# rosielab/emojivoice

Measured on AMD Instinct MI355X. Metric: audio_seconds_per_second, higher is better.
Workload: dtype f32 (deep layers: operand = two block-scaled fp16 pieces, product = 3 fp16 products on the fp16 MFMA, f32 accumulate); 1 GPU; config2: batch 64 x 516-frame (5.99 s) utterances per GPU, 10 Euler steps + HiFi-GAN V1, 22.05 kHz; global_batch=64, frames=516, ode_steps=10, parallelism=dp1, collective=none, batch_pipeline=cfm(i+1) || hifigan(i) on two streams, 2 pipeline(s) in flight

## Files before the change

emojivoice_amd/_lib.py:

```python
from __future__ import annotations

import ctypes as C
import os
import subprocess
from typing import Dict, Optional

import numpy as np
import torch

_HERE = os.path.dirname(os.path.abspath(__file__))
LIB_PATH = os.environ.get("EV_LIB_PATH") or os.path.join(_HERE, "lib", "libemojivoice_hip.so")
CSRC = os.path.join(_HERE, "csrc")

EXPORTS = [
    "ev_abi_version", "ev_create", "ev_destroy", "ev_last_error", "ev_load_estimator", "ev_load_vocoder", "ev_load_vocoder_cfg", "ev_load_text_encoder", "ev_text_encoder",
    "ev_text_encoder_status", "ev_stft_magnitude", "ev_denoise", "ev_align", "ev_dbg_conv_bench",
    "ev_workspace_bytes", "ev_cfm_decode", "ev_estimator", "ev_hifigan", "ev_profile_enable", "ev_profile_read", "ev_profile_read_split", "ev_dbg_last_cfg", "ev_set_arithmetic", "ev_get_arithmetic",
    "ev_op_conv1d", "ev_op_groupnorm_mish", "ev_op_groupnorm_mish2", "ev_op_conv_groupnorm", "ev_op_layernorm", "ev_op_split_pieces", "ev_op_attention", "ev_op_ln_mlp", "ev_set_mrf_streams_max",
    "ev_cfm_decode2", "ev_reserve", "ev_alloc_count", "ev_dbg_sk_stats", "ev_op_attn_out", "ev_dbg_set_amax", "ev_dbg_set_attn_h16", "ev_dbg_set_chain", "ev_dbg_sk_taken",
    "ev_load_mel_basis", "ev_mel_spectrogram",
    "ev_maximum_path", "ev_log_prior", "ev_mas_align",
    "ev_estimator_rows", "ev_cfm_loss",
    "ev_load_resampler", "ev_resample", "ev_mel_stats",
    "ev_trim_bounds", "ev_trim_apply",
    "ev_pitch_yin", "ev_dtw",
    "ev_loudness",
    "ev_pyin_observe", "ev_pyin_decode",
    "ev_op_attention2", "ev_op_attn_out2",
    "ev_load_stoi", "ev_stoi",
    "ev_load_stft_dist", "ev_stft_dist",
]


class EvLibraryError(RuntimeError):
# ... 116 lines not shown
    lib.ev_stft_dist.argtypes = [vp, vp, vp, vp, i32, i32, C.c_double, vp, vp, vp, vp]
    lib.ev_maximum_path.argtypes = [vp, vp, vp, vp, i32, i32, i32, vp, vp, vp]
    lib.ev_log_prior.argtypes = [vp, vp, vp, i32, i32, i32, vp, vp]
    lib.ev_mas_align.argtypes = [vp, vp, vp, vp, vp, i32, i32, i32, vp, vp, vp, vp, vp]
    lib.ev_profile_enable.argtypes = [vp, i32]
    lib.ev_profile_read.argtypes = [vp, C.POINTER(C.c_double), C.POINTER(C.c_double), C.POINTER(C.c_int64), i32]
    lib.ev_profile_read_split.argtypes = [vp, C.POINTER(C.c_double), C.POINTER(C.c_double), C.POINTER(C.c_int64)]
    lib.ev_dbg_last_cfg.argtypes = [vp]
    lib.ev_set_arithmetic.argtypes = [vp, i32]
    lib.ev_get_arithmetic.argtypes = [vp]
    lib.ev_dbg_set_amax.argtypes = [vp, i32]
    lib.ev_dbg_set_attn_h16.argtypes = [vp, i32]
    lib.ev_dbg_set_chain.argtypes = [vp, i32]
    lib.ev_dbg_sk_taken.argtypes = [vp]
    lib.ev_dbg_sk_taken.restype = C.c_int64
    lib.ev_op_conv1d.argtypes = [vp, vp, vp, vp, i32, i32, i32, i32, i32, i32, i32, i32, i32, f32, vp, vp]
    lib.ev_op_groupnorm_mish.argtypes = [vp, vp, vp, vp, vp, i32, i32, i32, i32, vp, vp]
    lib.ev_op_groupnorm_mish2.argtypes = [vp, vp, vp, vp, vp, i32, i32, i32, i32, i32, vp, i32, vp, vp, vp]
    lib.ev_op_conv_groupnorm.argtypes = [vp, vp, vp, vp, i32, i32, i32, vp, vp, vp, i32, vp, vp, vp, vp, vp, C.POINTER(C.c_int), vp]
    lib.ev_op_layernorm.argtypes = [vp, vp, vp, vp, i32, i32, vp, vp]
    lib.ev_op_split_pieces.argtypes = [vp, vp, i32, vp, vp]
    lib.ev_op_attention.argtypes = [vp, vp, vp, i32, i32, i32, vp, vp]
    lib.ev_op_attn_out.argtypes = [vp, vp, vp, i32, i32, vp, vp, vp, vp]
    lib.ev_op_attention2.argtypes = [vp, vp, vp, i32, i32, i32, i32, i32, i32, vp, C.POINTER(C.c_int), vp]
    lib.ev_op_attn_out2.argtypes = [vp, vp, vp, i32, i32, i32, i32, vp, vp, f32, f32, f32, vp, C.POINTER(C.c_int), vp]
    lib.ev_op_ln_mlp.argtypes = [vp, vp, vp, vp, vp, vp, vp, vp, vp, vp, vp, i32, i32, i32, vp, vp]
    for n in EXPORTS:
        getattr(lib, n)
    _lib = lib
    return lib
# ... 548 lines not shown
        self._check(self.lib.ev_op_split_pieces(self.h, x.data_ptr(), x.numel(), out.data_ptr(), _stream_ptr()), "ev_op_split_pieces")
        return out

    def set_arithmetic(self, bf16_products: int):
        self._check(self.lib.ev_set_arithmetic(self.h, int(bf16_products)), "ev_set_arithmetic")

    def set_amax(self, on: bool) -> None:
        self._check(self.lib.ev_dbg_set_amax(self.h, int(bool(on))), "ev_dbg_set_amax")

    def set_attn_h16(self, on: bool) -> None:
        self._check(self.lib.ev_dbg_set_attn_h16(self.h, int(bool(on))), "ev_dbg_set_attn_h16")

    def set_chain(self, on: bool) -> None:
        self._check(self.lib.ev_dbg_set_chain(self.h, int(bool(on))), "ev_dbg_set_chain")

    def arithmetic(self) -> int:
        return int(self.lib.ev_get_arithmetic(self.h))

    def last_cfg(self) -> int:
        return int(self.lib.ev_dbg_last_cfg(self.h))

    def profile_read_split(self):
        ms, fl, n = C.c_double(), C.c_double(), C.c_int64()
        self._check(self.lib.ev_profile_read_split(self.h, C.byref(ms), C.byref(fl), C.byref(n)), "ev_profile_read_split")
        return ms.value, fl.value, n.value

    def profile_read(self, reset: bool = True):
        ms, fl, n = C.c_double(), C.c_double(), C.c_int64()
        self._check(self.lib.ev_profile_read(self.h, C.byref(ms), C.byref(fl), C.byref(n), int(reset)), "ev_profile_read")
        return ms.value, fl.value, n.value
# ... 148 lines not shown
```

emojivoice_amd/csrc/ev_engine.hip:

```cpp
#include "ev_kernels.h"
#include "../../include/emojivoice.h"

#include <math.h>
#include <stdlib.h>
#include <stdarg.h>
#include <stdio.h>
#include <string.h>

#include <algorithm>
#include <atomic>
#include <mutex>
#include <numeric>
#include <string>
#include <unordered_map>
#include <vector>

namespace {

struct HostTensor {
    const float* p = nullptr;
    int ndim = 0;
    int64_t shape[4] = {0, 0, 0, 0};
    int64_t numel() const { int64_t n = 1; for (int i = 0; i < ndim; ++i) n *= shape[i]; return n; }
};
// ... 100 lines not shown
    Scratch stat_ws;
    Scratch trim_ws;
    Scratch loud_ws;
    Scratch stoi_ws;
    Scratch stftd_ws;
    float* zeros = nullptr;
    int max_steps = 64;
    int* bad_ids_host = nullptr; int* bad_ids_dev = nullptr;
    char* ws = nullptr; size_t ws_bytes = 0; size_t ws_used = 0; size_t ws_bytes_last = 0;
    int ws_B = -1, ws_Tp = -1, ws_Tv = -1;
    bool prof = false;
    bool fuse_pairs = true;
    bool fuse_attn = true;
    bool attn_h16 = true;
    bool use_chain = true;
    bool fuse_mlp = true;
    int gn_stats_tiles = 0;
    int fuse_mlp_min_tiles = 96;
    std::vector<hipEvent_t> ev_pool; size_t ev_used = 0;
    hipStream_t ws_stream = nullptr; bool ws_stream_valid = false;
    float* temb_host[2] = {nullptr, nullptr}; size_t temb_cap[2] = {0, 0}; hipEvent_t temb_ev[2] = {nullptr, nullptr}; int temb_slot = 0;
    float* cap_pool = nullptr; size_t cap_stride = 0; int cap_used = 0; int cap_nt[8] = {0};
    struct TprojEntry { int nt; float* d; };
    std::vector<TprojEntry> tproj_cache;
    bool captured = false; int cap_B = 0, cap_Tp = 0;
    int64_t n_allocs = 0;
    double prof_flops = 0; int64_t prof_launches = 0;
    struct ProfRec { int kind, Cin, Cout, ntaps, nrows, cfg, lean; double flops; bool split = false; };
    std::vector<ProfRec> prof_recs;
    hipStream_t stream = nullptr;
    hipStream_t mrf_stream[2] = {nullptr, nullptr};
    hipEvent_t mrf_ev[4] = {nullptr, nullptr, nullptr, nullptr};
    int ncu = 0;
    unsigned* sk_ctrl = nullptr;
    unsigned sk_seq = 0;
    float* sk_part = nullptr;
    int split_terms = 16;
    bool use_amax = true;
    bool amax_emitted = false;
    int n_fp32_only_layers = 0;
    int last_cfg = -1;
    bool sk_balance = true;
    int sk_wgs = 2;
// ... 289 lines not shown

template <auto Kernel>
inline void ensure_dyn_smem(size_t smem, int device) {
    static std::atomic<int> granted[16];
    static std::mutex slow[16];
    const int d = device & 15;
    if (smem <= 65536 || (int)smem <= granted[d].load(std::memory_order_acquire)) return;
    std::lock_guard<std::mutex> lk(slow[d]);
    const int cur = granted[d].load(std::memory_order_relaxed);
    if ((int)smem <= cur) return;
    if (hipFuncSetAttribute((const void*)Kernel, hipFuncAttributeMaxDynamicSharedMemorySize, (int)smem) == hipSuccess)
        granted[d].store((int)smem, std::memory_order_release);
    else (void)hipGetLastError();
}

template <auto Kernel, class Params>
inline void launch(int device, dim3 grid, dim3 block, size_t smem, hipStream_t st, const Params& p) {
    ensure_dyn_smem<Kernel>(smem, device);
    hipLaunchKernelGGL(Kernel, grid, block, smem, st, p);
}

template <int... Vs, class F>
inline void dispatch(int v, F&& f) { (void)((v == Vs && (f(std::integral_constant<int, Vs>{}), true)) || ...); }

constexpr int EPI_FULL = -1;
inline bool lean_acc(const ConvParams& p) { return p.accum || p.div3 || p.act2_lrelu; }
inline bool lean_ok(const ConvParams& p) {
    if (lean_acc(p) && (!p.R || p.act != ACT_NONE)) return false;
    return (p.act == ACT_NONE || p.act == ACT_LRELU || (p.act == ACT_SNAKE && (((size_t)p.act_a | (size_t)p.act_b) & 15) == 0)) &&
           ((!p.mask1 && !p.mask2) || (p.rowmask && p.mmul >= 1 && !(p.mask2 && lean_acc(p)))) && p.scale == 1.f &&
// ... 308 lines not shown
    p.Mpad = Lc.Mpad; p.Kpad = Lc.Kpad;
    p.Y = Y; p.ldy = C; p.Cout = C; p.osplit_log2 = 31; p.mmul = 1;
    p.nrows = g.nrows; p.S = g.S; p.P = g.P; p.T = g.T;
    p.pro_lrelu = 1; p.pro_slope = 0.1f;
    p.scale = 1.f; p.ldr = C; p.accum = e.accum; p.div3 = e.div3; p.act2_lrelu = e.act2_lrelu; p.act2_slope = e.act2_slope;
    p.yold = e.yold; p.ymax_mul = 1; h->amax_emitted = false;
    p.mtiles = 1; p.ntiles = (g.nrows + out_rows - 1) / out_rows;
}
inline void resblock_bounds(ev_handle* h, ConvParams& p, const Epi& e) {
    if (e.ymax && (!e.accum || e.yold) && h->use_amax) { p.ymax = e.ymax; h->amax_emitted = true; }
}

int launch_pair(ev_handle* h, const ConvLayer& L1, const ConvLayer& L2, const float* X, float* Y, int C, const Geom& g, const Epi& e) {
    if (over_4gib(g, C)) return fail(h, "tensor exceeds the 4 GiB buffer-addressing limit: split the batch");
    if (L1.sparse_taps || L2.sparse_taps || L1.Kpad != C || L2.Kpad != C || L1.Kpad != L2.Kpad || L1.Mpad != L2.Mpad || L1.halo_lo != L1.halo_hi ||
        L2.halo_lo != L2.halo_hi || 2 * L2.halo_lo > 16 || !L1.bias || !L2.bias)
        return fail(h, "launch_pair: unsupported layer pair");
    if (C != 32 && C != 64 && C != 128) return fail(h, "launch_pair: C must be 32, 64 or 128");
    PairParams pp;
    memset(&pp, 0, sizeof pp);
    ConvParams& p = pp.c2;
    const int NT = 8192 / C;
    pp.h1 = L1.halo_lo; pp.h2 = L2.halo_lo; pp.mid_slope = 0.1f; pp.out_rows = NT - 2 * pp.h2;
    resblock_params(h, p, L2, X, Y, C, g, e, pp.out_rows);
    p.W = L2.W; p.bias = L2.bias; p.ntaps = L2.ntaps; p.taplist = L2.taplist[0];
    p.R = X;
    pp.W1 = L1.W; pp.W1x = L1.Wx; p.Wx = L2.Wx; pp.W1h = L1.Wh; pp.w1h_scale = L1.wh_scale; p.Wh = L2.Wh; p.wh_scale = L2.wh_scale; pp.b1 = L1.bias; pp.taplist1 = L1.taplist[0]; pp.ntaps1 = L1.ntaps;
    if (prof_begin(h)) return 1;
    const int lean = epi_flavour(p, h->lean);
    const int split_terms = h->split_terms;
    const bool split = split_terms > 0 && lean != 0 && L1.Wx && L2.Wx && !(e.force_cfg == 0);
    const bool h16 = split && split_terms == 16 && L1.Wh && L2.Wh;
    const dim3 grid(p.ntiles), block(256);
    dispatch<32, 64, 128>(C, [&](auto CC) {
        constexpr int WM = CC / 32, WN = 4 / WM;
        if (h16) {
            resblock_bounds(h, p, e);
            const size_t smem = std::max((size_t)(NT + EV_HALO) * (4 * C + 16) + 64, (size_t)4 * 32 * 36 * sizeof(float));
            dispatch<1, 3>(lean, [&](auto E) { launch<resblock_pair_h16_kernel<WM, WN, E>>(h->device, grid, block, smem, h->stream, pp); });
        } else if (split) {
            const size_t rsb = 6 * C + 16;
            const size_t xs = (size_t)(NT + ((2 * pp.h1 + 7) & ~7)) * rsb, ys = (size_t)(NT + 16) * rsb, es = (size_t)4 * 32 * 36 * sizeof(float);
            const size_t smem = std::max(xs, std::max(ys, es));
            dispatch<1, 3>(lean, [&](auto E) {
                dispatch<3, 6>(split_terms == 3 ? 3 : 6, [&](auto TT) { launch<resblock_pair_split_kernel<WM, WN, E, TT>>(h->device, grid, block, smem, h->stream, pp); });
            });
        } else {
            const size_t xs = (size_t)(NT + ((2 * pp.h1 + 7) & ~7)) * EV_LDK, ys = (size_t)(C / 32) * (NT + 16) * EV_LDK, es = (size_t)4 * 32 * 36;
            const size_t smem = std::max(xs, std::max(ys, es)) * sizeof(float);
            dispatch<0, 1, 3>(lean, [&](auto E) { launch<resblock_pair_kernel<WM, WN, E>>(h->device, grid, block, smem, h->stream, pp); });
        }
    });
    HIPCHK(h, hipGetLastError());
    const int code = (h16 ? 160 : split ? 140 : 100) + L2.ntaps;
    h->last_cfg = code;
    return h->prof ? prof_end(h, {1, C, C, L1.ntaps, g.nrows, code, lean, 2.0 * (L1.macs_per_row + L2.macs_per_row) * valid_rows(g), split}) : 0;
}

inline int chain_halo(const ConvLayer* L1, const ConvLayer* L2) { int hs = 0; for (int m = 0; m < 3; ++m) hs += L1[m].halo_lo + L2[m].halo_lo; return hs; }
inline bool chain_ok(const ev_handle* h, const ConvLayer* L1, const ConvLayer* L2, int C) {
    if (!h->use_chain || h->split_terms != 16 || (C != 32 && C != 64)) return false;
    int hb = 0;
    for (int m = 0; m < 3; ++m) {
        const ConvLayer &a = L1[m], &b = L2[m];
        if (!a.Wh || !b.Wh || !a.bias || !b.bias || a.sparse_taps || b.sparse_taps || a.Kpad != C || b.Kpad != C || a.Mpad != b.Mpad || a.Mpad != L1[0].Mpad ||
            a.halo_lo != a.halo_hi || b.halo_lo != b.halo_hi || a.ntaps != L1[0].ntaps || b.ntaps != L2[0].ntaps || a.ntaps > 64 || b.ntaps > 64) return false;
        hb = std::max(hb, std::max(a.halo_lo, b.halo_lo));
    }
    const int NT = C == 32 ? 256 : 128, hs = chain_halo(L1, L2);
    return hs <= 12 && 2 * hb <= EV_HALO && NT - 2 * hs >= NT / 2;
}
// ... 5 lines not shown
    int hb = 0;
    double macs = 0;
    for (int m = 0; m < 3; ++m) {
        cp.W1h[m] = L1[m].Wh; cp.W2h[m] = L2[m].Wh; cp.w1_scale[m] = L1[m].wh_scale; cp.w2_scale[m] = L2[m].wh_scale;
        cp.b1[m] = L1[m].bias; cp.b2[m] = L2[m].bias; cp.tl1[m] = L1[m].taplist[0]; cp.tl2[m] = L2[m].taplist[0];
        hb = std::max(hb, std::max(L1[m].halo_lo, L2[m].halo_lo));
        macs += L1[m].macs_per_row + L2[m].macs_per_row;
    }
    cp.ntaps1 = L1[0].ntaps; cp.ntaps2 = L2[0].ntaps; cp.hb = hb; cp.halo = chain_halo(L1, L2); cp.mid_slope = 0.1f;
    const int NT = 8192 / C;
    cp.out_rows = NT - 2 * cp.halo;
    resblock_params(h, p, L2[2], X, Y, C, g, e, cp.out_rows);
    resblock_bounds(h, p, e);
    if (prof_begin(h)) return 1;
    const int lean = epi_flavour(p, true);
    const size_t smem = std::max((size_t)(NT + EV_HALO) * (4 * C + 16) + 64, (size_t)4 * 32 * 36 * sizeof(float));
    dispatch<32, 64>(C, [&](auto CC) {
        constexpr int WM = CC / 32, WN = 4 / WM;
        dispatch<1, 3>(lean, [&](auto E) { launch<resblock_chain_h16_kernel<WM, WN, E>>(h->device, dim3(p.ntiles), dim3(256), smem, h->stream, cp); });
    });
    HIPCHK(h, hipGetLastError());
    h->last_cfg = 180 + L2[0].ntaps;
    return h->prof ? prof_end(h, {1, C, C, L1[0].ntaps, g.nrows, 180 + L2[0].ntaps, lean, 2.0 * macs * valid_rows(g), true}) : 0;
}

inline int rb2_halo(const ConvLayer* L) { return L[0].halo_lo + L[1].halo_lo; }
inline bool rb2_ok(const ev_handle* h, const ConvLayer* L, int C) {
    if (!h->use_chain || h->split_terms != 16 || (C != 32 && C != 64 && C != 128)) return false;
    for (int m = 0; m < 2; ++m) {
        const ConvLayer& a = L[m];
        if (!a.Wh || !a.bias || a.sparse_taps || a.Kpad != C || a.Mpad != L[0].Mpad || a.halo_lo != a.halo_hi || a.ntaps != L[0].ntaps || a.ntaps > 64) return false;
    }
    const int NT = C == 32 ? 256 : C == 64 ? 128 : 64;
    return 8 * (NT - 2 * rb2_halo(L)) >= h->rb2_minkeep * NT && NT - 2 * rb2_halo(L) > 0;
// ... 4 lines not shown
    memset(&cp, 0, sizeof cp);
    ConvParams& p = cp.c2;
    int hb = 0;
    for (int m = 0; m < 2; ++m) {
        cp.Wh[m] = L[m].Wh; cp.w_scale[m] = L[m].wh_scale; cp.b[m] = L[m].bias; cp.tl[m] = L[m].taplist[0];
        hb = std::max(hb, L[m].halo_lo);
    }
    cp.ntaps = L[0].ntaps; cp.hb = hb; cp.halo = rb2_halo(L);
    const int NT = 8192 / C;
    cp.out_rows = NT - 2 * cp.halo;
    if (cp.out_rows <= 0) return fail(h, "launch_rb2: halo %d leaves no row of a %d-frame tile", cp.halo, NT);
    resblock_params(h, p, L[1], X, Y, C, g, e, cp.out_rows);
    resblock_bounds(h, p, e);
    if (prof_begin(h)) return 1;
    const int lean = epi_flavour(p, true);
    const size_t smem = std::max((size_t)(NT + 2 * hb) * (4 * C + 16) + 64, (size_t)4 * 32 * 36 * sizeof(float));
    dispatch<32, 64, 128>(C, [&](auto CC) {
        constexpr int WM = CC / 32, WN = 4 / WM;
        dispatch<1, 3>(lean, [&](auto E) { launch<resblock2_h16_kernel<WM, WN, E>>(h->device, dim3(p.ntiles), dim3(256), smem, h->stream, cp); });
    });
    HIPCHK(h, hipGetLastError());
    h->last_cfg = 200 + L[0].ntaps;
    return h->prof ? prof_end(h, {1, C, C, L[0].ntaps, g.nrows, 200 + L[0].ntaps, lean, 2.0 * (L[0].macs_per_row + L[1].macs_per_row) * valid_rows(g), true}) : 0;
}

int launch_gn(ev_handle* h, const float* X, int ldx, float* Y, int ldy, const float* gamma, const float* beta, const float* rowmask,
              const float* temb, const float* R, int ldr, const Geom& g, int C, int mode, const float* part = nullptr, int temb_stride = 0) {
    GNParams p;
    p.X = X; p.ldx = ldx; p.Y = Y; p.ldy = ldy; p.gamma = gamma; p.beta = beta; p.rowmask = rowmask; p.temb = temb; p.R = R; p.ldr = ldr;
    p.S = g.S; p.P = g.P; p.T = g.T; p.CG = C / 8; p.mode = mode; p.eps = 1e-5f; p.temb_stride = temb_stride;
    if (p.CG != 32) return fail(h, "groupnorm kernel expects 32 channels per group, got %d", p.CG);
// ... 773 lines not shown

int ev_create(ev_handle** out, int device, const ev_model_dims* dims) {
    if (!out || !dims) return 1;
    *out = nullptr;
    int ndev = 0;
    if (hipGetDeviceCount(&ndev) != hipSuccess || device < 0 || device >= ndev) return 2;
    if (hipSetDevice(device) != hipSuccess) return 3;
    ev_handle* h = new ev_handle();
    h->device = device;
    h->dims = *dims;
    { const char* fp = getenv("EV_FUSE_PAIRS"); if (fp && *fp == '0') h->fuse_pairs = false; }
    { const char* fp = getenv("EV_FUSE_MLP"); if (fp && *fp == '0') h->fuse_mlp = false; }
    { const char* fp = getenv("EV_FUSE_ATTN"); if (fp && *fp == '0') h->fuse_attn = false; }
    if (getenv("EV_NO_ATTN_H16")) h->attn_h16 = false;
    if (getenv("EV_NO_CHAIN")) h->use_chain = false;
    { const char* fp = getenv("EV_FUSE_MLP_MIN"); if (fp && *fp) h->fuse_mlp_min_tiles = atoi(fp); }
    { const char* fp = getenv("EV_MRF_STREAMS_MAX"); if (fp && *fp) h->mrf_max_frames = atoi(fp); }
    if (getenv("EV_NO_AMAX")) h->use_amax = false;
    { const char* sp = getenv("EV_SPLIT"); if (sp && *sp) { const int t = atoi(sp); h->split_terms = (t == 0 || t == 3 || t == 6 || t == 9 || t == 16) ? t : 16; } }
    { const char* fp = getenv("EV_NO_SK_BALANCE"); if (fp && *fp && *fp != '0') h->sk_balance = false; }
    { const char* fp = getenv("EV_SK_SPIN"); if (fp && *fp) h->sk_spin = atoi(fp); }
    { const char* fp = getenv("EV_SK_WGS"); if (fp && *fp) h->sk_wgs = std::min(3, std::max(1, atoi(fp))); }
    { const char* fp = getenv("EV_FORCE_CFG"); if (fp && *fp) h->force_cfg = atoi(fp); }
    if (getenv("EV_NO_LEAN")) h->lean = false;
    if (getenv("EV_NO_SK")) h->small_sk = false;
    if (getenv("EV_NO_SK32_LEAN")) h->sk32_lean = false;
    if (getenv("EV_NO_GN_STATS")) h->gn_stats = false;
    if (getenv("EV_NO_QKV_H16")) h->qkv_h16 = false;
    if (getenv("EV_NO_ATTN_SK")) h->attn_sk = false;
    { const char* fp = getenv("EV_ATTN_TPW"); if (fp) h->attn_tpw = std::max(1, atoi(fp)); }
// ... 1354 lines not shown
                if (l < nl) with_slots(e2, x, nullptr, y, 1);
                if (launch_chain(h, w.c1[i * 3 + j], w.c2[i * 3 + j], x, y, C, v.g[l], e2)) return 1;
                wrote(y, e2.accum != 0);
                if (ms) HIPCHK(h, hipEventRecord(h->mrf_ev[j], h->stream));
                continue;
            }
            for (int mm = 0; mm < 3; ++mm) {
                if (ms && mm == 2 && j > 0) HIPCHK(h, hipStreamWaitEvent(h->stream, h->mrf_ev[j - 1], 0));
                Epi e2; e2.R = x; e2.ldr = C;
                float* y = pp[mm & 1];
                if (mm == 2) {
                    y = v.XS[l];
                    e2.accum = (j > 0);
                    if (j == 2) { e2.div3 = 1; e2.act2_lrelu = 1; e2.act2_slope = next_slope; }
                }
                if (h->fuse_pairs && (C == 32 || C == 64 || (C == 128 && w.c1[i * 3 + j][mm].ntaps <= 3))) {
                    if (mm == 2 && l < nl) with_slots(e2, x, nullptr, y, 1);
                    if (launch_pair(h, w.c1[i * 3 + j][mm], w.c2[i * 3 + j][mm], x, y, C, v.g[l], e2)) return 1;
                    wrote(y, e2.accum != 0);
                } else {
                    Epi e1; e1.pro_slope = 0.1f; e1.act = ACT_LRELU; e1.act_slope = 0.1f;
                    with_slots(e1, x, nullptr, t1, 1);
                    if (launch_conv(h, w.c1[i * 3 + j][mm], x, C, t1, C, v.g[l], e1)) return 1;
                    wrote(t1, false);
                    with_slots(e2, t1, x, y, 1);
                    if (launch_conv(h, w.c2[i * 3 + j][mm], t1, C, y, C, v.g[l], e2)) return 1;
                    wrote(y, e2.accum != 0);
                }
                if (ms && mm == 2) HIPCHK(h, hipEventRecord(h->mrf_ev[j], h->stream));
                x = y;
            }
// ... 39 lines not shown
    for (size_t i = 0; i + 1 < h->ev_used; i += 2) {
        float t = 0;
        HIPCHK(h, hipEventElapsedTime(&t, h->ev_pool[i], h->ev_pool[i + 1]));
        ms += t;
    }
    if (const char* dump = getenv("EV_PROFILE_DUMP")) {
        if (*dump && h->prof_recs.size() * 2 == h->ev_used) {
            struct Agg { ev_handle::ProfRec r; double ms = 0, fl = 0; int n = 0; };
            std::vector<Agg> aggs;
            for (size_t i = 0; i < h->prof_recs.size(); ++i) {
                const auto& r = h->prof_recs[i];
                float t = 0;
                hipEventElapsedTime(&t, h->ev_pool[2 * i], h->ev_pool[2 * i + 1]);
                Agg* a = nullptr;
                for (auto& x : aggs)
                    if (x.r.kind == r.kind && x.r.Cin == r.Cin && x.r.Cout == r.Cout && x.r.ntaps == r.ntaps && x.r.nrows == r.nrows && x.r.cfg == r.cfg && x.r.lean == r.lean) a = &x;
                if (!a) { aggs.push_back(Agg{r}); a = &aggs.back(); }
                a->ms += t; a->fl += r.flops; a->n += 1;
            }
            if (FILE* f = fopen(dump, "a")) {
                fprintf(f, "# kind Cin Cout ntaps nrows cfg lean launches total_ms TFLOP/s\n");
                for (auto& a : aggs)
                    fprintf(f, "%s %4d %4d %3d %9d %3d %d %5d %9.3f %7.1f\n", a.r.kind == 0 ? "conv" : (a.r.kind == 1 ? "pair" : (a.r.kind == 2 ? "lnff" : (a.r.kind == 3 ? "lnqkv" : "attn "))), a.r.Cin, a.r.Cout, a.r.ntaps, a.r.nrows, a.r.cfg, a.r.lean,
                            a.n, a.ms, a.fl / (a.ms * 1e9));
                fclose(f);
            }
        }
    }
    if (conv_ms) *conv_ms = ms;
    if (conv_flops) *conv_flops = h->prof_flops;
    if (conv_launches) *conv_launches = h->prof_launches;
    if (reset) { h->ev_used = 0; h->prof_flops = 0; h->prof_launches = 0; h->prof_recs.clear(); }
    return 0;
}

int ev_dbg_last_cfg(ev_handle* h) { return h ? h->last_cfg : -1; }

int ev_set_arithmetic(ev_handle* h, int bf16_products) {
    if (!h) return 1;
// ... 1 lines not shown
        return fail(h, "ev_set_arithmetic: 0, 3, 6, 9 or 16, got %d", bf16_products);
    h->split_terms = bf16_products;
    return 0;
}
int ev_get_arithmetic(ev_handle* h) { return h ? h->split_terms : -1; }

int ev_dbg_set_amax(ev_handle* h, int on) {
    if (!h) return 1;
    h->use_amax = on != 0;
    return 0;
}

int ev_dbg_set_chain(ev_handle* h, int on) {
    if (!h) return 1;
    h->use_chain = on != 0;
    return 0;
}

int ev_dbg_set_attn_h16(ev_handle* h, int on) {
    if (!h) return 1;
    h->attn_h16 = on != 0;
    return 0;
}

int ev_profile_read_split(ev_handle* h, double* ms_out, double* flops_out, int64_t* launches_out) {
    if (!h) return 1;
    HIPCHK(h, hipStreamSynchronize(h->stream));
    double ms = 0, fl = 0;
    int64_t n = 0;
    if (h->prof_recs.size() * 2 == h->ev_used)
// ... 414 lines not shown
```

emojivoice_amd/csrc/ev_kernels.h:

```cpp
#pragma once
#include <hip/hip_runtime.h>
#include <stdint.h>
#include <type_traits>

typedef float f32x16 __attribute__((ext_vector_type(16)));
typedef float f32x4 __attribute__((ext_vector_type(4)));
typedef int i32x4 __attribute__((ext_vector_type(4)));

#define EV_MAX_TAPS 16
#define EV_BK 32
#define EV_LDK 36
#define EV_WROWS 128
#define EV_SK_MAXF4(TW) ((TW) == 4 ? (64 + 64) * 8 * 8 : 16 * 512)
#define EV_HALO 64

enum { ACT_NONE = 0, ACT_LRELU = 1, ACT_TANH = 2, ACT_SILU = 3, ACT_MISH = 4, ACT_SNAKE = 5 };

struct SkCtl {
    unsigned* ctrl;
    unsigned* flags;
    float* part;
    int part_floats;
    int q, r;
    int spin_limit;
// ... 2238 lines not shown
            }
        }
    };
    conv_epilogue_lean<1, 1, LEAN>(p, accs, smem, m0, n0, lane, -0x7fffffff, 0x7fffffff, reduce);
    if ((p.dbg & 16) && tid == 0) p.stamps[4 * wg + 3] = __builtin_amdgcn_s_memrealtime();
}

struct PairParams {
    ConvParams c2;
    const float* W1; const float* b1; const int2* taplist1; int ntaps1;
    const void* W1h; float w1h_scale;
    const void* W1x;
    int h1, h2;
    float mid_slope;
    int out_rows;
};

template <int WAVES_M, int WAVES_N, int LEAN = 0>
__global__ __launch_bounds__(256, WAVES_M == 2 ? 4 : 3) void resblock_pair_kernel(const PairParams pp) {
    constexpr int TM = 1, TN = 2;
    constexpr int NT = WAVES_N * TN * 32;
    constexpr int NCH = WAVES_M;
    constexpr int XROWS = NT + EV_HALO;
    constexpr int YROWS = NT + 16;
    constexpr int XPASS = XROWS / 32;
    static_assert(WAVES_M * WAVES_N == 4, "4 waves per workgroup");
    const ConvParams& p = pp.c2;
    extern __shared__ __attribute__((aligned(16))) float smem[];
    float* Xs = smem;
    float* Ys = smem;
// ... 131 lines not shown
            const int row = br < pp.h2 ? br : NT + br;
            f32x4 z = {0.f, 0.f, 0.f, 0.f};
            *(f32x4*)(Ys + (chn * YROWS + row) * EV_LDK + c4) = z;
        }
    }
    ev_lds_barrier();

    phase(p.W, p.taplist, p.ntaps, LEAN ? p.bias : nullptr, [&](int ch) -> const float* {
        return Ys + (ch * YROWS + wn * (TN * 32) + li + pp.h2) * EV_LDK + 4 * lh;
    });

    if constexpr (LEAN != 0) conv_epilogue_lean<TM, TN, LEAN>(p, acc, smem + wave * (32 * (TM * 32 + 4)), wm * 32, g0 + wn * (TN * 32), lane, n0, n0 + pp.out_rows);
    else conv_epilogue<TM, TN, false>(p, acc, smem + wave * (32 * (TM * 32 + 4)), wm * 32, g0 + wn * (TN * 32), lane, n0, n0 + pp.out_rows);
}

template <int WAVES_M, int WAVES_N, class PIPE>
struct EvResblockCore {
    static constexpr int TM = 1, TN = 2;
    static constexpr int C = 32 * WAVES_M;
    static constexpr int NT = WAVES_N * TN * 32;
    static constexpr int PIECES = PIPE::PIECES;
    static constexpr unsigned KGB = PIPE::KG_BYTES;
    static constexpr int RSB = PIECES * 2 * C + 16;
    static constexpr int NS = C / 16, H = NS / 2;
    static_assert(WAVES_M * WAVES_N == 4, "4 waves per workgroup");

    char* Xb;
    float* red;
    int tid, lane, wave, wm, wn, li, lh;
    unsigned wlane, wbase;
// ... 232 lines not shown
                char* dst = Xb + (r + pp.h2) * RSB + (wm * 32 + 8 * g + 4 * lh) * 2;
                *(uint2*)(dst) = q0v; *(uint2*)(dst + 2 * C) = q1v; *(uint2*)(dst + 4 * C) = q2v;
            }
        }
        k.template zero_border_rows<6 * C / 16>(pp.h2);
    }
    k.acc_init(LEAN ? p.bias : pp.b1, 1.f);
    ev_lds_barrier();

    k.kloop(rW2, tlv2, ng2, k.bbase(pp.h2));

    conv_epilogue_lean<TM, TN, LEAN>(p, k.acc, smem + wave * (32 * (TM * 32 + 4)), wm * 32, g0 + k.row0(), lane, n0, n0 + pp.out_rows);
}

template <int WAVES_M, int WAVES_N, int LEAN>
__global__ __launch_bounds__(256, 2) void resblock_pair_h16_kernel(const PairParams pp) {
    using Core = EvResblockCore<WAVES_M, WAVES_N, EvPipeH16>;
    constexpr int TM = Core::TM, TN = Core::TN, C = Core::C, NT = Core::NT, RSB = Core::RSB, H = Core::H;
    constexpr int TPR = C / 4, RPS = 256 / TPR;
    constexpr int XPASS = (NT + EV_HALO) / RPS;
    const ConvParams& p = pp.c2;
    extern __shared__ __attribute__((aligned(16))) float smem[];

    const int nt = ev_xcd_remap(blockIdx.x, p.ntiles);
    const int n0 = nt * pp.out_rows;
    const int g0 = n0 - pp.h2;
    if (ev_tile_is_padding(p.S, p.P, p.T, p.nrows, n0, pp.out_rows)) return;
    Core k((char*)smem, smem + ((NT + EV_HALO) * RSB) / 4, p.Kpad);
    char* Xb = k.Xb;
    const int tid = k.tid, lane = k.lane, wave = k.wave, wm = k.wm;
    const int srow = tid / TPR, sc4 = (tid % TPR) * 4;
    const int nw0 = g0 + k.row0();
    EvAmax am = ev_amax_begin(p, nw0, TN * 32);
    const __amdgpu_buffer_rsrc_t rX = ev_rsrc(p.X);

    const __amdgpu_buffer_rsrc_t rW1 = ev_rsrc(pp.W1h), rW2 = ev_rsrc(p.Wh);
    const int ng1 = pp.ntaps1 * H, ng2 = p.ntaps * H;
    const int2 tlv1 = (lane < pp.ntaps1) ? pp.taplist1[lane] : make_int2(0, 0);
    const int2 tlv2 = (lane < p.ntaps) ? p.taplist[lane] : make_int2(0, 0);
    k.ring_fill(rW1, tlv1, ng1);
    float sx;
    {
        const int xrows = NT + 2 * pp.h1;
// ... 62 lines not shown
    }
    ev_amax_from_acc<TM, TN>(p, am, k.acc, nw0, lane);
    conv_epilogue_lean<TM, TN, LEAN>(p, k.acc, smem + wave * (32 * (TM * 32 + 4)), wm * 32, nw0, lane, n0, n0 + pp.out_rows);
    ev_amax_emit(p, am, nw0, TN * 32, lane);
}

struct ChainParams {
    ConvParams c2;
    const void* W1h[3]; const void* W2h[3]; float w1_scale[3], w2_scale[3];
    const float* b1[3]; const float* b2[3];
    const int2* tl1[3]; const int2* tl2[3];
    int ntaps1, ntaps2;
    int hb;
    int halo;
    int out_rows;
    float mid_slope;
};
template <int WAVES_M, int WAVES_N, int LEAN>
__global__ __launch_bounds__(256, 2) void resblock_chain_h16_kernel(const ChainParams cp) {
    using Core = EvResblockCore<WAVES_M, WAVES_N, EvPipeH16>;
    constexpr int TN = Core::TN, C = Core::C, NT = Core::NT, RSB = Core::RSB, H = Core::H;
    static_assert(C == 32 || C == 64, "C = 32 / 64");
    const ConvParams& p = cp.c2;
    extern __shared__ __attribute__((aligned(16))) float smem[];
    const int nt = ev_xcd_remap(blockIdx.x, p.ntiles);
    const int n0 = nt * cp.out_rows;
    const int g0 = n0 - cp.halo;
    if (ev_tile_is_padding(p.S, p.P, p.T, p.nrows, n0, cp.out_rows)) return;
    Core k((char*)smem, smem + ((NT + EV_HALO) * RSB) / 4, p.Kpad);
    const int lane = k.lane;
    EvAmax am = ev_amax_begin(p, g0 + k.row0(), TN * 32);
    f32x16 xr[TN];
    float inside[TN];
    k.running_x_load(p, g0, cp.hb, xr, inside);
    const int ng1 = cp.ntaps1 * H, ng2 = cp.ntaps2 * H;
#pragma unroll 1
    for (int m = 0; m < 3; ++m) {
        const __amdgpu_buffer_rsrc_t rW1 = ev_rsrc(cp.W1h[m]), rW2 = ev_rsrc(cp.W2h[m]);
        const int2 tlv1 = (lane < cp.ntaps1) ? cp.tl1[m][lane] : make_int2(0, 0);
        const int2 tlv2 = (lane < cp.ntaps2) ? cp.tl2[m][lane] : make_int2(0, 0);
        k.ring_fill(rW1, tlv1, ng1);
        k.acc_from_lrelu_x(xr, p.pro_slope);
        const float u1 = k.conv_from_acc(0, cp.hb, rW1, tlv1, ng1, cp.b1[m], cp.w1_scale[m]);
        k.ring_fill(rW2, tlv2, ng2);
// ... 19 lines not shown
    int hb;
    int halo;
    int out_rows;
};
template <int WAVES_M, int WAVES_N, int LEAN>
__global__ __launch_bounds__(256, 2) void resblock2_h16_kernel(const Rb2Params cp) {
    using Core = EvResblockCore<WAVES_M, WAVES_N, EvPipeH16>;
    constexpr int TN = Core::TN, C = Core::C, NT = Core::NT, RSB = Core::RSB, H = Core::H;
    static_assert(C == 32 || C == 64 || C == 128, "C = 32 / 64 / 128");
    const ConvParams& p = cp.c2;
    extern __shared__ __attribute__((aligned(16))) float smem[];
    const int nt = ev_xcd_remap(blockIdx.x, p.ntiles);
    const int n0 = nt * cp.out_rows;
    const int g0 = n0 - cp.halo;
    if (ev_tile_is_padding(p.S, p.P, p.T, p.nrows, n0, cp.out_rows)) return;
    Core k((char*)smem, smem + ((NT + 2 * cp.hb) * RSB) / 4, p.Kpad);
    const int lane = k.lane;
    EvAmax am = ev_amax_begin(p, g0 + k.row0(), TN * 32);
    f32x16 xr[TN];
    float inside[TN];
    k.running_x_load(p, g0, cp.hb, xr, inside);
    const int ng = cp.ntaps * H;
#pragma unroll 1
    for (int m = 0; m < 2; ++m) {
        const __amdgpu_buffer_rsrc_t rW = ev_rsrc(cp.Wh[m]);
        const int2 tlv = (lane < cp.ntaps) ? cp.tl[m][lane] : make_int2(0, 0);
        k.ring_fill(rW, tlv, ng);
        k.acc_from_lrelu_x(xr, p.pro_slope);
        const float u = k.conv_from_acc(4 * m, cp.hb, rW, tlv, ng, cp.b[m], cp.w_scale[m]);
        k.running_x_add(xr, inside, u);
    }
// ... 4070 lines not shown
```

include/emojivoice.h:

```cpp
#ifndef EMOJIVOICE_H
#define EMOJIVOICE_H

#include <stddef.h>
#include <stdint.h>

#ifdef __cplusplus
extern "C" {
#endif

#define EV_ABI_VERSION 4

typedef struct ev_handle ev_handle;

typedef struct ev_tensor_index {
    const char *name;
    uint64_t offset;
    int32_t ndim;
    int64_t shape[4];
} ev_tensor_index;

typedef struct ev_model_dims {
    int32_t n_feats;
    int32_t spk_emb_dim;
    int32_t channels;
// ... 117 lines not shown
                 double *d_frame , double *d_sums , int32_t *d_counts , void *stream);

int ev_profile_enable(ev_handle *h, int on);
int ev_profile_read(ev_handle *h, double *conv_ms, double *conv_flops, int64_t *conv_launches, int reset);
int ev_profile_read_split(ev_handle *h, double *ms, double *flops, int64_t *launches);
int ev_set_arithmetic(ev_handle *h, int setting);
int ev_get_arithmetic(ev_handle *h);

int ev_dbg_last_cfg(ev_handle *h);

int ev_dbg_conv_bench(ev_handle *h, int Cin, int Cout, int K, int dil, int B, int T, int P, int iters, int dbg, int cfg, float *ms_out);

int ev_dbg_set_amax(ev_handle *h, int on);
int ev_dbg_set_attn_h16(ev_handle *h, int on);
int ev_dbg_set_chain(ev_handle *h, int on);

int ev_dbg_sk_stats(ev_handle *h, uint32_t *out3);
int64_t ev_dbg_sk_taken(ev_handle *h);

int ev_op_conv1d(ev_handle *h, const float *d_x , const float *w ,
                 const float *bias , int B, int Cin, int T, int Cout, int K, int dilation,
                 int transposed, int stride, int padding, float pre_lrelu_slope , float *d_y, void *stream);
int ev_op_groupnorm_mish(ev_handle *h, const float *d_x , const float *d_gamma, const float *d_beta,
                         const int32_t *d_lengths, int B, int C, int T, int groups, float *d_y, void *stream);
int ev_op_groupnorm_mish2(ev_handle *h, const float *d_x , const float *d_gamma, const float *d_beta,
                          const int32_t *d_lengths, int B, int C, int T, int groups, int mode, const float *d_temb,
                          int temb_stride, const float *d_R, float *d_y, void *stream);
int ev_op_conv_groupnorm(ev_handle *h, const float *d_x , const float *w ,
                         const float *bias , int Cin, int T, int K, const float *d_gamma,
                         const float *d_beta, const int32_t *d_lengths , int mode, const float *d_temb, const float *d_R,
// ... 23 lines not shown
```

Measured before the change: 4729 audio_s/s.

## Size resblock pair/chain LDS to the actual halo to raise occupancy

The fused HiFi-GAN resblock pair and chain kernels used to reserve LDS for the worst-case halo (NT + EV_HALO rows). The launcher now computes the exact row count from the layer halos, queries the occupancy of the exact and padded sizes, and passes the chosen tile_rows to the kernel so its reduction area sits right after the tile. Launch bounds for the pair kernel are raised from 2 to 3 or 4 workgroups per CU so that more resident workgroups are possible. The risk is register pressure or spilling under the tighter launch bounds. A debug export, env knobs, and halo fields in the profile records are also added.

```diff
diff --git a/emojivoice_amd/_lib.py b/emojivoice_amd/_lib.py
--- a/emojivoice_amd/_lib.py
+++ b/emojivoice_amd/_lib.py
@@ -18,6 +18,7 @@
     "ev_workspace_bytes", "ev_cfm_decode", "ev_estimator", "ev_hifigan", "ev_profile_enable", "ev_profile_read", "ev_profile_read_split", "ev_dbg_last_cfg", "ev_set_arithmetic", "ev_get_arithmetic",
     "ev_op_conv1d", "ev_op_groupnorm_mish", "ev_op_groupnorm_mish2", "ev_op_conv_groupnorm", "ev_op_layernorm", "ev_op_split_pieces", "ev_op_attention", "ev_op_ln_mlp", "ev_set_mrf_streams_max",
     "ev_cfm_decode2", "ev_reserve", "ev_alloc_count", "ev_dbg_sk_stats", "ev_op_attn_out", "ev_dbg_set_amax", "ev_dbg_set_attn_h16", "ev_dbg_set_chain", "ev_dbg_sk_taken",
+    "ev_dbg_pair_lds",
     "ev_load_mel_basis", "ev_mel_spectrogram",
     "ev_maximum_path", "ev_log_prior", "ev_mas_align",
     "ev_estimator_rows", "ev_cfm_loss",
@@ -164,6 +165,7 @@
     lib.ev_dbg_set_chain.argtypes = [vp, i32]
     lib.ev_dbg_sk_taken.argtypes = [vp]
     lib.ev_dbg_sk_taken.restype = C.c_int64
+    lib.ev_dbg_pair_lds.argtypes = [vp, i32, i32, i32, i32, i32, C.POINTER(C.c_int)]
     lib.ev_op_conv1d.argtypes = [vp, vp, vp, vp, i32, i32, i32, i32, i32, i32, i32, i32, i32, f32, vp, vp]
     lib.ev_op_groupnorm_mish.argtypes = [vp, vp, vp, vp, vp, i32, i32, i32, i32, vp, vp]
     lib.ev_op_groupnorm_mish2.argtypes = [vp, vp, vp, vp, vp, i32, i32, i32, i32, i32, vp, i32, vp, vp, vp]
@@ -742,6 +744,11 @@
     def set_chain(self, on: bool) -> None:
         self._check(self.lib.ev_dbg_set_chain(self.h, int(bool(on))), "ev_dbg_set_chain")
 
+    def pair_lds(self, C_: int, h1: int, h2: int, mode: int = 2, lean: int = 1):
+        out = (C.c_int * 4)()
+        self._check(self.lib.ev_dbg_pair_lds(self.h, int(C_), int(lean), int(h1), int(h2), int(mode), out), "ev_dbg_pair_lds")
+        return tuple(int(v) for v in out)
+
     def arithmetic(self) -> int:
         return int(self.lib.ev_get_arithmetic(self.h))
 
diff --git a/emojivoice_amd/csrc/ev_engine.hip b/emojivoice_amd/csrc/ev_engine.hip
--- a/emojivoice_amd/csrc/ev_engine.hip
+++ b/emojivoice_amd/csrc/ev_engine.hip
@@ -138,6 +138,8 @@
     bool fuse_attn = true;
     bool attn_h16 = true;
     bool use_chain = true;
+    bool exact_lds = true;
+    int fuse128_taps = 3;
     bool fuse_mlp = true;
     int gn_stats_tiles = 0;
     int fuse_mlp_min_tiles = 96;
@@ -150,7 +152,7 @@
     bool captured = false; int cap_B = 0, cap_Tp = 0;
     int64_t n_allocs = 0;
     double prof_flops = 0; int64_t prof_launches = 0;
-    struct ProfRec { int kind, Cin, Cout, ntaps, nrows, cfg, lean; double flops; bool split = false; };
+    struct ProfRec { int kind, Cin, Cout, ntaps, nrows, cfg, lean; double flops; bool split = false; int halo = 0; };
     std::vector<ProfRec> prof_recs;
     hipStream_t stream = nullptr;
     hipStream_t mrf_stream[2] = {nullptr, nullptr};
@@ -470,6 +472,33 @@
     else (void)hipGetLastError();
 }
 
+template <auto Kernel>
+inline int wgs_per_cu(size_t smem, int device) {
+    struct Known { int device; size_t smem; int wgs; };
+    static std::mutex mu;
+    static std::vector<Known> known;
+    std::lock_guard<std::mutex> lk(mu);
+    for (const Known& k : known) if (k.device == device && k.smem == smem) return k.wgs;
+    ensure_dyn_smem<Kernel>(smem, device);
+    int n = 0;
+    if (hipOccupancyMaxActiveBlocksPerMultiprocessor(&n, (const void*)Kernel, 256, smem) != hipSuccess) { (void)hipGetLastError(); n = 0; }
+    known.push_back({device, smem, n});
+    return n;
+}
+
+struct RbLds { int rows = 0; size_t bytes = 0; int wgs = 0; };
+template <auto Kernel>
+inline RbLds rb_lds(const ev_handle* h, int C, int hb, int mode) {
+    const int NT = 8192 / C;
+    RbLds exact, padded;
+    exact.rows = ev_rb_rows(NT, hb); padded.rows = std::max(NT + EV_HALO, exact.rows);
+    exact.bytes = (size_t)ev_rb_h16_lds_bytes(C, exact.rows); padded.bytes = (size_t)ev_rb_h16_lds_bytes(C, padded.rows);
+    padded.wgs = wgs_per_cu<Kernel>(padded.bytes, h->device);
+    if (mode == 1 || (mode == 2 && !h->exact_lds)) return padded;
+    exact.wgs = wgs_per_cu<Kernel>(exact.bytes, h->device);
+    return (mode == 0 || exact.wgs > padded.wgs) ? exact : padded;
+}
+
 template <auto Kernel, class Params>
 inline void launch(int device, dim3 grid, dim3 block, size_t smem, hipStream_t st, const Params& p) {
     ensure_dyn_smem<Kernel>(smem, device);
@@ -808,7 +837,7 @@
 int launch_pair(ev_handle* h, const ConvLayer& L1, const ConvLayer& L2, const float* X, float* Y, int C, const Geom& g, const Epi& e) {
     if (over_4gib(g, C)) return fail(h, "tensor exceeds the 4 GiB buffer-addressing limit: split the batch");
     if (L1.sparse_taps || L2.sparse_taps || L1.Kpad != C || L2.Kpad != C || L1.Kpad != L2.Kpad || L1.Mpad != L2.Mpad || L1.halo_lo != L1.halo_hi ||
-        L2.halo_lo != L2.halo_hi || 2 * L2.halo_lo > 16 || !L1.bias || !L2.bias)
+        L2.halo_lo != L2.halo_hi || 2 * L2.halo_lo > 16 || 2 * L1.halo_lo > EV_HALO || !L1.bias || !L2.bias)
         return fail(h, "launch_pair: unsupported layer pair");
     if (C != 32 && C != 64 && C != 128) return fail(h, "launch_pair: C must be 32, 64 or 128");
     PairParams pp;
@@ -830,8 +859,11 @@
         constexpr int WM = CC / 32, WN = 4 / WM;
         if (h16) {
             resblock_bounds(h, p, e);
-            const size_t smem = std::max((size_t)(NT + EV_HALO) * (4 * C + 16) + 64, (size_t)4 * 32 * 36 * sizeof(float));
-            dispatch<1, 3>(lean, [&](auto E) { launch<resblock_pair_h16_kernel<WM, WN, E>>(h->device, grid, block, smem, h->stream, pp); });
+            dispatch<1, 3>(lean, [&](auto E) {
+                const RbLds lds = rb_lds<resblock_pair_h16_kernel<WM, WN, E>>(h, C, ev_rb_pair_hb(pp.h1, pp.h2), 2);
+                pp.tile_rows = lds.rows;
+                launch<resblock_pair_h16_kernel<WM, WN, E>>(h->device, grid, block, lds.bytes, h->stream, pp);
+            });
         } else if (split) {
             const size_t rsb = 6 * C + 16;
             const size_t xs = (size_t)(NT + ((2 * pp.h1 + 7) & ~7)) * rsb, ys = (size_t)(NT + 16) * rsb, es = (size_t)4 * 32 * 36 * sizeof(float);
@@ -848,7 +880,7 @@
     HIPCHK(h, hipGetLastError());
     const int code = (h16 ? 160 : split ? 140 : 100) + L2.ntaps;
     h->last_cfg = code;
-    return h->prof ? prof_end(h, {1, C, C, L1.ntaps, g.nrows, code, lean, 2.0 * (L1.macs_per_row + L2.macs_per_row) * valid_rows(g), split}) : 0;
+    return h->prof ? prof_end(h, {1, C, C, L1.ntaps, g.nrows, code, lean, 2.0 * (L1.macs_per_row + L2.macs_per_row) * valid_rows(g), split, pp.h1}) : 0;
 }
 
 inline int chain_halo(const ConvLayer* L1, const ConvLayer* L2) { int hs = 0; for (int m = 0; m < 3; ++m) hs += L1[m].halo_lo + L2[m].halo_lo; return hs; }
@@ -884,10 +916,13 @@
     resblock_bounds(h, p, e);
     if (prof_begin(h)) return 1;
     const int lean = epi_flavour(p, true);
-    const size_t smem = std::max((size_t)(NT + EV_HALO) * (4 * C + 16) + 64, (size_t)4 * 32 * 36 * sizeof(float));
     dispatch<32, 64>(C, [&](auto CC) {
         constexpr int WM = CC / 32, WN = 4 / WM;
-        dispatch<1, 3>(lean, [&](auto E) { launch<resblock_chain_h16_kernel<WM, WN, E>>(h->device, dim3(p.ntiles), dim3(256), smem, h->stream, cp); });
+        dispatch<1, 3>(lean, [&](auto E) {
+            const RbLds lds = rb_lds<resblock_chain_h16_kernel<WM, WN, E>>(h, C, hb, 2);
+            cp.tile_rows = lds.rows;
+            launch<resblock_chain_h16_kernel<WM, WN, E>>(h->device, dim3(p.ntiles), dim3(256), lds.bytes, h->stream, cp);
+        });
     });
     HIPCHK(h, hipGetLastError());
     h->last_cfg = 180 + L2[0].ntaps;
@@ -922,7 +957,7 @@
     resblock_bounds(h, p, e);
     if (prof_begin(h)) return 1;
     const int lean = epi_flavour(p, true);
-    const size_t smem = std::max((size_t)(NT + 2 * hb) * (4 * C + 16) + 64, (size_t)4 * 32 * 36 * sizeof(float));
+    const size_t smem = (size_t)ev_rb_h16_lds_bytes(C, ev_rb_rows(NT, hb));
     dispatch<32, 64, 128>(C, [&](auto CC) {
         constexpr int WM = CC / 32, WN = 4 / WM;
         dispatch<1, 3>(lean, [&](auto E) { launch<resblock2_h16_kernel<WM, WN, E>>(h->device, dim3(p.ntiles), dim3(256), smem, h->stream, cp); });
@@ -1726,6 +1761,8 @@
     { const char* fp = getenv("EV_FUSE_ATTN"); if (fp && *fp == '0') h->fuse_attn = false; }
     if (getenv("EV_NO_ATTN_H16")) h->attn_h16 = false;
     if (getenv("EV_NO_CHAIN")) h->use_chain = false;
+    { const char* fp = getenv("EV_PAD_LDS"); if (fp && *fp && *fp != '0') h->exact_lds = false; }
+    { const char* fp = getenv("EV_FUSE128_TAPS"); if (fp && *fp) h->fuse128_taps = atoi(fp); }
     { const char* fp = getenv("EV_FUSE_MLP_MIN"); if (fp && *fp) h->fuse_mlp_min_tiles = atoi(fp); }
     { const char* fp = getenv("EV_MRF_STREAMS_MAX"); if (fp && *fp) h->mrf_max_frames = atoi(fp); }
     if (getenv("EV_NO_AMAX")) h->use_amax = false;
@@ -3110,7 +3147,7 @@
                     e2.accum = (j > 0);
                     if (j == 2) { e2.div3 = 1; e2.act2_lrelu = 1; e2.act2_slope = next_slope; }
                 }
-                if (h->fuse_pairs && (C == 32 || C == 64 || (C == 128 && w.c1[i * 3 + j][mm].ntaps <= 3))) {
+                if (h->fuse_pairs && (C == 32 || C == 64 || (C == 128 && w.c1[i * 3 + j][mm].ntaps <= h->fuse128_taps))) {
                     if (mm == 2 && l < nl) with_slots(e2, x, nullptr, y, 1);
                     if (launch_pair(h, w.c1[i * 3 + j][mm], w.c2[i * 3 + j][mm], x, y, C, v.g[l], e2)) return 1;
                     wrote(y, e2.accum != 0);
@@ -3180,15 +3217,15 @@
                 hipEventElapsedTime(&t, h->ev_pool[2 * i], h->ev_pool[2 * i + 1]);
                 Agg* a = nullptr;
                 for (auto& x : aggs)
-                    if (x.r.kind == r.kind && x.r.Cin == r.Cin && x.r.Cout == r.Cout && x.r.ntaps == r.ntaps && x.r.nrows == r.nrows && x.r.cfg == r.cfg && x.r.lean == r.lean) a = &x;
+                    if (x.r.kind == r.kind && x.r.Cin == r.Cin && x.r.Cout == r.Cout && x.r.ntaps == r.ntaps && x.r.nrows == r.nrows && x.r.cfg == r.cfg && x.r.lean == r.lean && x.r.halo == r.halo) a = &x;
                 if (!a) { aggs.push_back(Agg{r}); a = &aggs.back(); }
                 a->ms += t; a->fl += r.flops; a->n += 1;
             }
             if (FILE* f = fopen(dump, "a")) {
-                fprintf(f, "# kind Cin Cout ntaps nrows cfg lean launches total_ms TFLOP/s\n");
+                fprintf(f, "# kind Cin Cout ntaps nrows cfg lean launches total_ms TFLOP/s c1_halo\n");
                 for (auto& a : aggs)
-                    fprintf(f, "%s %4d %4d %3d %9d %3d %d %5d %9.3f %7.1f\n", a.r.kind == 0 ? "conv" : (a.r.kind == 1 ? "pair" : (a.r.kind == 2 ? "lnff" : (a.r.kind == 3 ? "lnqkv" : "attn "))), a.r.Cin, a.r.Cout, a.r.ntaps, a.r.nrows, a.r.cfg, a.r.lean,
-                            a.n, a.ms, a.fl / (a.ms * 1e9));
+                    fprintf(f, "%s %4d %4d %3d %9d %3d %d %5d %9.3f %7.1f %3d\n", a.r.kind == 0 ? "conv" : (a.r.kind == 1 ? "pair" : (a.r.kind == 2 ? "lnff" : (a.r.kind == 3 ? "lnqkv" : "attn "))), a.r.Cin, a.r.Cout, a.r.ntaps, a.r.nrows, a.r.cfg, a.r.lean,
+                            a.n, a.ms, a.fl / (a.ms * 1e9), a.r.halo);
                 fclose(f);
             }
         }
@@ -3220,6 +3257,23 @@
 int ev_dbg_set_chain(ev_handle* h, int on) {
     if (!h) return 1;
     h->use_chain = on != 0;
+    return 0;
+}
+
+int ev_dbg_pair_lds(ev_handle* h, int C, int lean, int h1, int h2, int mode, int* out) {
+    if (!h || !out) return 1;
+    if ((C != 32 && C != 64 && C != 128) || (lean != 1 && lean != 3) || h1 < 0 || h2 < 0 || 2 * h1 > EV_HALO || 2 * h2 > 16 || mode < 0 || mode > 2)
+        return fail(h, "ev_dbg_pair_lds: C = %d, lean = %d, h1 = %d, h2 = %d, mode = %d not supported", C, lean, h1, h2, mode);
+    HIPCHK(h, hipSetDevice(h->device));
+    RbLds lds;
+    dispatch<32, 64, 128>(C, [&](auto CC) {
+        constexpr int WM = CC / 32, WN = 4 / WM;
+        dispatch<1, 3>(lean, [&](auto E) { lds = rb_lds<resblock_pair_h16_kernel<WM, WN, E>>(h, C, ev_rb_pair_hb(h1, h2), mode); });
+    });
+    int per_cu = 0;
+    HIPCHK(h, hipDeviceGetAttribute(&per_cu, hipDeviceAttributeMaxSharedMemoryPerMultiprocessor, h->device));
+    if (lds.wgs <= 0) return fail(h, "ev_dbg_pair_lds: the occupancy query failed");
+    out[0] = lds.rows; out[1] = (int)lds.bytes; out[2] = lds.wgs; out[3] = per_cu;
     return 0;
 }
 
diff --git a/emojivoice_amd/csrc/ev_kernels.h b/emojivoice_amd/csrc/ev_kernels.h
--- a/emojivoice_amd/csrc/ev_kernels.h
+++ b/emojivoice_amd/csrc/ev_kernels.h
@@ -2276,6 +2276,7 @@
     int h1, h2;
     float mid_slope;
     int out_rows;
+    int tile_rows;
 };
 
 template <int WAVES_M, int WAVES_N, int LEAN = 0>
@@ -2437,6 +2438,16 @@
     else conv_epilogue<TM, TN, false>(p, acc, smem + wave * (32 * (TM * 32 + 4)), wm * 32, g0 + wn * (TN * 32), lane, n0, n0 + pp.out_rows);
 }
 
+__host__ __device__ constexpr int ev_rb_rows(int NT, int hb) { return NT + 2 * hb; }
+__host__ __device__ constexpr int ev_rb_pair_hb(int h1, int h2) { return h1 > h2 ? h1 : h2; }
+__host__ __device__ constexpr int ev_rb_h16_rsb(int C) { return 4 * C + 16; }
+__host__ __device__ constexpr int ev_rb_h16_red_off(int C, int rows) { return rows * ev_rb_h16_rsb(C); }
+__host__ __device__ constexpr int ev_rb_h16_lds_bytes(int C, int rows) {
+    const int tile = ev_rb_h16_red_off(C, rows) + 16 * (int)sizeof(float), epi = 4 * 32 * 36 * (int)sizeof(float);
+    return tile > epi ? tile : epi;
+}
+static_assert(ev_rb_h16_lds_bytes(32, 256 + EV_HALO) == 46144 && ev_rb_h16_lds_bytes(128, 64 + EV_HALO) == 67648, "the padded request of the earlier builds");
+
 template <int WAVES_M, int WAVES_N, class PIPE>
 struct EvResblockCore {
     static constexpr int TM = 1, TN = 2;
@@ -2699,7 +2710,7 @@
 }
 
 template <int WAVES_M, int WAVES_N, int LEAN>
-__global__ __launch_bounds__(256, 2) void resblock_pair_h16_kernel(const PairParams pp) {
+__global__ __launch_bounds__(256, WAVES_M == 4 ? 3 : 4) void resblock_pair_h16_kernel(const PairParams pp) {
     using Core = EvResblockCore<WAVES_M, WAVES_N, EvPipeH16>;
     constexpr int TM = Core::TM, TN = Core::TN, C = Core::C, NT = Core::NT, RSB = Core::RSB, H = Core::H;
     constexpr int TPR = C / 4, RPS = 256 / TPR;
@@ -2711,7 +2722,8 @@
     const int n0 = nt * pp.out_rows;
     const int g0 = n0 - pp.h2;
     if (ev_tile_is_padding(p.S, p.P, p.T, p.nrows, n0, pp.out_rows)) return;
-    Core k((char*)smem, smem + ((NT + EV_HALO) * RSB) / 4, p.Kpad);
+    static_assert(RSB == ev_rb_h16_rsb(C), "one LDS layout for kernel and launcher");
+    Core k((char*)smem, smem + ev_rb_h16_red_off(C, pp.tile_rows) / 4, p.Kpad);
     char* Xb = k.Xb;
     const int tid = k.tid, lane = k.lane, wave = k.wave, wm = k.wm;
     const int srow = tid / TPR, sc4 = (tid % TPR) * 4;
@@ -2804,6 +2816,7 @@
     int hb;
     int halo;
     int out_rows;
+    int tile_rows;
     float mid_slope;
 };
 template <int WAVES_M, int WAVES_N, int LEAN>
@@ -2817,7 +2830,8 @@
     const int n0 = nt * cp.out_rows;
     const int g0 = n0 - cp.halo;
     if (ev_tile_is_padding(p.S, p.P, p.T, p.nrows, n0, cp.out_rows)) return;
-    Core k((char*)smem, smem + ((NT + EV_HALO) * RSB) / 4, p.Kpad);
+    static_assert(RSB == ev_rb_h16_rsb(C), "one LDS layout for kernel and launcher");
+    Core k((char*)smem, smem + ev_rb_h16_red_off(C, cp.tile_rows) / 4, p.Kpad);
     const int lane = k.lane;
     EvAmax am = ev_amax_begin(p, g0 + k.row0(), TN * 32);
     f32x16 xr[TN];
@@ -2867,7 +2881,8 @@
     const int n0 = nt * cp.out_rows;
     const int g0 = n0 - cp.halo;
     if (ev_tile_is_padding(p.S, p.P, p.T, p.nrows, n0, cp.out_rows)) return;
-    Core k((char*)smem, smem + ((NT + 2 * cp.hb) * RSB) / 4, p.Kpad);
+    static_assert(RSB == ev_rb_h16_rsb(C), "one LDS layout for kernel and launcher");
+    Core k((char*)smem, smem + ev_rb_h16_red_off(C, ev_rb_rows(NT, cp.hb)) / 4, p.Kpad);
     const int lane = k.lane;
     EvAmax am = ev_amax_begin(p, g0 + k.row0(), TN * 32);
     f32x16 xr[TN];
diff --git a/include/emojivoice.h b/include/emojivoice.h
--- a/include/emojivoice.h
+++ b/include/emojivoice.h
@@ -155,6 +155,7 @@
 int ev_dbg_set_amax(ev_handle *h, int on);
 int ev_dbg_set_attn_h16(ev_handle *h, int on);
 int ev_dbg_set_chain(ev_handle *h, int on);
+int ev_dbg_pair_lds(ev_handle *h, int C, int lean, int h1, int h2, int mode, int *out4);
 
 int ev_dbg_sk_stats(ev_handle *h, uint32_t *out3);
 int64_t ev_dbg_sk_taken(ev_handle *h);
```

Result: no change. 4763 audio_s/s, median of 6 (+0.7%).
